# microsoft/DirectXTex

Measured on AMD Instinct MI355X. Metric: Mtexels/s BC7 encode (4096^2 RGBA8, TEX_COMPRESS_DEFAULT), higher is better.
Workload: dtype fp32 seed fit + i32 exact error sums (u8 texels in, 128-bit blocks out); 1 GPU; cfg2: 4096x4096 RGBA8 -> BC7_UNORM, TEX_COMPRESS_DEFAULT, one image per GPU, source and payload resident in HBM (dxtex_compress_device)

## Files before the change

directxtex_amd/csrc/bc6h_encode.hip:

```cpp
#include "dxtex_kernels.h"
#include "bc67_tables.h"
#include "bc7_core.h"
#include "bc6h_core.h"
#include "search_common.h"
#include <algorithm>
#include <cstdlib>
#include <cstdio>
#include <vector>

namespace dxtex
{
namespace
{
using namespace bc6h;

struct Ep16 { uint32_t a01, a2b0, b12; };
__device__ __forceinline__ Ep16 pack_ep16(const int (&A)[3], const int (&B)[3])
{
    Ep16 e;
    e.a01 = (uint32_t(A[0]) & 0xFFFFu) | (uint32_t(A[1]) << 16);
    e.a2b0 = (uint32_t(A[2]) & 0xFFFFu) | (uint32_t(B[0]) << 16);
    e.b12 = (uint32_t(B[1]) & 0xFFFFu) | (uint32_t(B[2]) << 16);
    return e;
}
// ... 14 lines not shown
__device__ __forceinline__ PkState pk_pack(const Perturb6& s)
{
    PkState p; p.ep = pack_ep16(s.ep.A, s.ep.B); p.err = s.err; p.err0 = s.err0;
    p.misc = (uint32_t(s.new0) & 0xFFFFu) | (uint32_t(s.ch) << 16) | (uint32_t(s.sub) << 18) | (uint32_t(s.do_b) << 20);
    return p;
}
__device__ __forceinline__ Perturb6 pk_unpack(const PkState& p, bool sg)
{
    Perturb6 s; unpack_ep16(p.ep, sg, s.ep.A, s.ep.B); s.err = p.err; s.err0 = p.err0;
    s.new0 = int(int16_t(p.misc & 0xFFFFu)); s.ch = int((p.misc >> 16) & 3u); s.sub = int((p.misc >> 18) & 3u); s.do_b = int((p.misc >> 20) & 1u);
    return s;
}
struct Rec6 { Ep16 ep; float err; };
struct Best6 { float err; uint32_t mode; uint64_t lo, hi; };
struct OrgSave { Ep16 ep; float err; uint64_t idx; };
struct OptSave { uint64_t idx; float err; uint32_t swapped; };

enum : int { SEED_INTS = 17 * 6 + 2 };

struct Bc6hArgs
{
    SegTable seg;
    uint32_t nblocks;
    int isSigned;
    int prune;
    uint32_t taskBase;
    int prec1[4];
    float* fpix;
    uint8_t* lists;
    int* seeds;
    Rec6* recs;
    OrgSave* orgs;
    uint2* order; uint32_t* tinfo; uint32_t* counters;
    Best6* best;
    float* bounds;
    int boundsReady;
    int filterStats;
    int samePrec;
    struct OptSave* opts;
    int saveOpt;
    ModeRt mode;
};

constexpr uint32_t kDoneBit6 = 1u << 23;

#if !defined(DXTEX_BC6H_DEFAULT_ORDER)
#define DXTEX_BC6H_DEFAULT_ORDER "5,6,7,8,0,2,3,4,1,9"
#endif

__device__ __forceinline__ Texels slot_texels(float* slot , int np)
{
    Texels t; t.r = slot; t.g = slot + 16 * 64; t.b = slot + 32 * 64; t.stride = 64; t.np = np;
    return t;
}

__device__ __forceinline__ int gather_texels(const float* planes, uint32_t mask, float* slot, uint64_t& pos)
{
    int np = 0; pos = 0;
#pragma unroll
    for (int i = 0; i < 16; ++i)
        if ((mask >> i) & 1u)
        {
            slot[np * 64] = planes[i]; slot[(16 + np) * 64] = planes[16 + i]; slot[(32 + np) * 64] = planes[32 + i];
            pos |= uint64_t(i) << (4 * np);
            ++np;
        }
// ... 901 lines not shown
        const float tr = gp[0], tg = gp[16], tb = gp[32];
        EndPts e;
        unpack_ep16(rec.ep, sg, e.A, e.B);
        Perturb6 st = perturb6_begin(e, rec.err);
        while (st.ch < 3)
        {
            float err; int v;
            perturb6_wave_macro(tr, tg, tb, lane, st, prec, sg, err, v);
            st = perturb6_transition(st, err, v);
        }
        if (lane == 0)
        {
            a.recs[myTask].ep = pack_ep16(st.ep.A, st.ep.B);
            { const float mk = ep16_mark(sg, st.ep.A, st.ep.B); if (mk < 0.0f) a.recs[myTask].err = mk; }
        }
    }
}

__global__ void __launch_bounds__(256) bc6h_store_kernel(Bc6hArgs a)
{
    const uint32_t nb = blockIdx.x * 256u + threadIdx.x;
    if (nb >= a.nblocks) return;
    const Best6 b = a.best[nb];
    const BcSeg& im = seg_of(a.seg, nb);
    const uint32_t gb = im.nb0 + (nb - im.l0);
    const uint32_t by = gb / im.nbw, bx = gb - by * im.nbw;
    uint64_t* out = reinterpret_cast<uint64_t*>(im.dst + uint64_t(by) * im.dstRowPitch) + 2 * uint64_t(bx);
    out[0] = b.lo; out[1] = b.hi;
}

const uint64_t kMaxBlocksPerPass6 = dev_env("DXTEX_MAX_BLOCKS_PER_PASS") ? std::max<uint64_t>(1, strtoull(dev_env("DXTEX_MAX_BLOCKS_PER_PASS"), nullptr, 10)) : (1u << 22);
struct Scratch6
{
    size_t fpix, lists, seeds, recs, orgs, order, tinfo, counters, best, bounds, recs1, orgs1, order1, tinfo1, counters1, opts, total;
    explicit Scratch6(uint64_t nb)
    {
        auto up = [](size_t v) { return (v + 255) & ~size_t(255); };
        size_t o = 0;
        fpix = o; o = up(o + nb * 48 * sizeof(float));
        lists = o; o = up(o + nb * 8);
        seeds = o; o = up(o + nb * SEED_INTS * sizeof(int));
        recs = o; o = up(o + nb * 16 * sizeof(Rec6));
        orgs = o; o = up(o + nb * 16 * sizeof(OrgSave));
        order = o; o = up(o + nb * 16 * sizeof(uint2));
        tinfo = o; o = up(o + nb * 16 * sizeof(uint32_t));
        counters = o; o = up(o + 128 * sizeof(uint32_t));
        best = o; o = up(o + nb * sizeof(Best6));
        bounds = o; o = up(o + nb * 17 * sizeof(float));
        recs1 = o; o = up(o + nb * 4 * sizeof(Rec6));
        orgs1 = o; o = up(o + nb * 4 * sizeof(OrgSave));
        order1 = o; o = up(o + nb * 4 * sizeof(uint2));
        tinfo1 = o; o = up(o + nb * 4 * sizeof(uint32_t));
        counters1 = o; o = up(o + 128 * sizeof(uint32_t));
        opts = o; o = up(o + nb * 16 * sizeof(OptSave));
        total = o;
    }
};
}

size_t bc6h_scratch_bytes(uint64_t nblocks, size_t nimages)
{
    return Scratch6(nblocks < kMaxBlocksPerPass6 ? nblocks : kMaxBlocksPerPass6).total + seg_table_bytes(nblocks, kMaxBlocksPerPass6, nimages);
}

hipError_t launch_bc6h_encode(const SrcView& src, uint8_t* dst, uint64_t dstRowPitch, bool isSigned, void* scratch,
                              hipStream_t stream, KernelMarks* marks, const SideStreams* side)
{
    BcImage one; one.src = src; one.dst = dst; one.dstRowPitch = dstRowPitch;
    return launch_bc6h_encode_many(&one, 1, isSigned, scratch, stream, marks, side);
}

hipError_t launch_bc6h_encode_many(const BcImage* images, size_t count, bool isSigned, void* scratch, hipStream_t stream, KernelMarks* marks,
                                   const SideStreams* side)
{
#define DXTEX_MARK(NAME) do { if (marks) marks->mark(NAME); } while (0)
    std::vector<BcSeg> segs;
    std::vector<BcPass> passes;
    uint64_t perPass = 0;
    if (!build_passes(images, count, kMaxBlocksPerPass6, segs, passes, &perPass)) return hipSuccess;
    const Scratch6 L(perPass);
    uint8_t* base = static_cast<uint8_t*>(scratch);
    BcSeg* dSegs = reinterpret_cast<BcSeg*>(base + L.total);
    const hipError_t ce = upload_segments(dSegs, segs, passes, stream);
    if (ce != hipSuccess) return ce;
    for (const BcPass& pass : passes)
    {
        Bc6hArgs a;
        set_pass(a.seg, dSegs, segs, pass);
        a.nblocks = pass.nblocks;
        a.isSigned = isSigned ? 1 : 0;
        static const bool noPrune = dev_env("DXTEX_BC6H_NO_PRUNE") != nullptr;
        a.prune = noPrune ? 0 : 1;
        a.fpix = reinterpret_cast<float*>(base + L.fpix);
        a.lists = base + L.lists;
        a.seeds = reinterpret_cast<int*>(base + L.seeds);
        a.recs = reinterpret_cast<Rec6*>(base + L.recs);
        a.orgs = reinterpret_cast<OrgSave*>(base + L.orgs);
        a.order = reinterpret_cast<uint2*>(base + L.order);
        a.tinfo = reinterpret_cast<uint32_t*>(base + L.tinfo);
        a.counters = reinterpret_cast<uint32_t*>(base + L.counters);
        a.best = reinterpret_cast<Best6*>(base + L.best);
        a.bounds = reinterpret_cast<float*>(base + L.bounds);
        a.opts = reinterpret_cast<OptSave*>(base + L.opts);
        a.saveOpt = 0;
        a.boundsReady = 0;
        a.filterStats = 0;
        a.mode = ModeRt();

        DXTEX_MARK("bc6h_rough");
        hipLaunchKernelGGL(bc6h_rough_kernel, dim3((a.nblocks + 3) / 4), dim3(256), 0, stream, a);
        DXTEX_MARK("bc6h_block_seed");
        hipLaunchKernelGGL(bc6h_block_seed_kernel, dim3((a.nblocks + 255) / 256), dim3(256), 0, stream, a);
        if (dev_env("DXTEX_BC6H_DUMP"))
        {
            (void)hipStreamSynchronize(stream);
            const uint32_t n = std::min<uint32_t>(a.nblocks, 4);
            std::vector<uint8_t> l(n * 8); std::vector<int> sd(n * SEED_INTS);
            (void)hipMemcpy(l.data(), a.lists, l.size(), hipMemcpyDeviceToHost);
            (void)hipMemcpy(sd.data(), a.seeds, sd.size() * 4, hipMemcpyDeviceToHost);
            for (uint32_t b = 0; b < n; ++b)
            {
                fprintf(stderr, "block %u shapes:", b);
                for (int i = 0; i < 8; ++i) fprintf(stderr, " %d", l[b * 8 + i]);
                fprintf(stderr, "\n  seeds rank0:");
                for (int i = 0; i < 12; ++i) fprintf(stderr, " %d", sd[b * SEED_INTS + i]);
                fprintf(stderr, "\n");
            }
        }
        static const int onlyMode = dev_env("DXTEX_BC6H_ONLY_MODE") ? atoi(dev_env("DXTEX_BC6H_ONLY_MODE")) : -1;
        static const bool noSearch = dev_env("DXTEX_BC6H_NO_SEARCH") != nullptr;
        static const Bc6hMode kModes[14] = {
            { 0x00, 1, 1, 3, { 10, 10, 10 }, { 5, 5, 5 } }, { 0x01, 1, 1, 3, { 7, 7, 7 }, { 6, 6, 6 } }, { 0x02, 1, 1, 3, { 11, 11, 11 }, { 5, 4, 4 } },
            { 0x06, 1, 1, 3, { 11, 11, 11 }, { 4, 5, 4 } }, { 0x0a, 1, 1, 3, { 11, 11, 11 }, { 4, 4, 5 } }, { 0x0e, 1, 1, 3, { 9, 9, 9 }, { 5, 5, 5 } },
            { 0x12, 1, 1, 3, { 8, 8, 8 }, { 6, 5, 5 } }, { 0x16, 1, 1, 3, { 8, 8, 8 }, { 5, 6, 5 } }, { 0x1a, 1, 1, 3, { 8, 8, 8 }, { 5, 5, 6 } },
            { 0x1e, 1, 0, 3, { 6, 6, 6 }, { 6, 6, 6 } }, { 0x03, 0, 0, 4, { 10, 10, 10 }, { 10, 10, 10 } }, { 0x07, 0, 1, 4, { 11, 11, 11 }, { 9, 9, 9 } },
            { 0x0b, 0, 1, 4, { 12, 12, 12 }, { 8, 8, 8 } }, { 0x0f, 0, 1, 4, { 16, 16, 16 }, { 4, 4, 4 } } };
        auto set_mode_on = [&](Bc6hArgs& a, int mi)
        {
            const Bc6hMode& k = kModes[mi];
            a.mode.index = mi; a.mode.code = k.code; a.mode.regions2 = k.regions2; a.mode.transformed = k.transformed; a.mode.prec = k.prec[0];
            for (int c = 0; c < 3; ++c) a.mode.delta[c] = k.delta[c];
        };
        auto set_mode = [&](int mi) { set_mode_on(a, mi); };
        auto sort_tasks = [&](const Bc6hArgs& a, uint32_t ntasks, hipStream_t stream)
        {
            const uint32_t binGroups = std::min<uint32_t>(kBinGroups, (ntasks + 255) / 256);
            (void)hipMemsetAsync(a.counters, 0, 128 * sizeof(uint32_t), stream);
            hipLaunchKernelGGL(bc7_bin_count_kernel, dim3(binGroups), dim3(256), 0, stream, a.tinfo, ntasks, a.counters);
            hipLaunchKernelGGL(bc7_bin_scan_kernel, dim3(1), dim3(1), 0, stream, a.counters);
            hipLaunchKernelGGL(bc7_bin_scatter_kernel, dim3(binGroups), dim3(256), 0, stream, a.tinfo, ntasks, a.counters, a.order);
        };
        a.taskBase = 0;
        for (int m = 0; m < 4; ++m) a.prec1[m] = kModes[10 + m].prec[0];
        static const std::vector<int> order6 = []
        {
            std::vector<int> o;
            const char* e = dev_env("DXTEX_BC6H_ORDER");
            const char* p = e ? e : DXTEX_BC6H_DEFAULT_ORDER;
            while (*p) { if (*p >= '0' && *p <= '9') o.push_back(int(strtol(p, const_cast<char**>(&p), 10))); else ++p; }
            return o;
        }();
        int prevPrec = -1;
        a.samePrec = 0;
        std::vector<int> run2;
        for (int mi : order6) if (mi >= 0 && mi <= 9 && (onlyMode < 0 || mi == onlyMode)) run2.push_back(mi);
        static const int forkBack = dev_env("DXTEX_BC6H_FORK_BACK") ? atoi(dev_env("DXTEX_BC6H_FORK_BACK")) : 2;
        const SideStreams* fork = (marks || forkBack <= 0 || run2.size() < size_t(forkBack) + 1 || onlyMode >= 0) ? nullptr : side;
        Bc6hArgs a1 = a;
        a1.recs = reinterpret_cast<Rec6*>(base + L.recs1);
        a1.orgs = reinterpret_cast<OrgSave*>(base + L.orgs1);
        a1.order = reinterpret_cast<uint2*>(base + L.order1);
        a1.tinfo = reinterpret_cast<uint32_t*>(base + L.tinfo1);
        a1.counters = reinterpret_cast<uint32_t*>(base + L.counters1);
        a1.samePrec = 0;
        auto one_region_search = [&](hipStream_t stream, KernelMarks* marks)
        {
            const uint32_t gridPP = (a1.nblocks + 255) / 256;
            DXTEX_MARK("bc6h_pre_1region");
            a1.boundsReady = 0;
            for (int m = 0; m < 4; ++m)
            {
                if (onlyMode >= 0 && 10 + m != onlyMode) continue;
                set_mode_on(a1, 10 + m); a1.taskBase = uint32_t(m) * a1.nblocks;
                hipLaunchKernelGGL(bc6h_pre_kernel<0>, dim3(gridPP), dim3(256), 0, stream, a1);
                a1.boundsReady = 1;
            }
            const uint32_t ntasks = a1.nblocks * 4u;
            if (onlyMode >= 0)
                for (int m = 0; m < 4; ++m) if (10 + m != onlyMode) (void)hipMemsetAsync(a1.tinfo + uint64_t(m) * a1.nblocks, 0, uint64_t(a1.nblocks) * 4, stream);
            DXTEX_MARK("bc6h_bin_1region");
            sort_tasks(a1, ntasks, stream);
            DXTEX_MARK("bc6h_perturb_1region");
            static const uint32_t waveMax = dev_env("DXTEX_BC6H_WAVE_MAX") ? uint32_t(strtoul(dev_env("DXTEX_BC6H_WAVE_MAX"), nullptr, 0)) : kWaveTaskMax6;
            if (!noSearch)
            {
                hipLaunchKernelGGL(bc6h_perturb_kernel<16>, dim3(std::min<uint32_t>(kSearchWaves, (ntasks + 63) / 64)), dim3(64), 0, stream, a1, waveMax);
                hipLaunchKernelGGL(bc6h_perturb_wave_kernel, dim3(std::min<uint32_t>(kSearchWaves, ntasks)), dim3(64), 0, stream, a1, waveMax);
            }
        };
        bool forked = false;
        for (size_t at = 0; at < run2.size(); ++at)
        {
            const int mi = run2[at];
            if (fork && at + size_t(forkBack) == run2.size())
            {
                (void)hipEventRecord(fork->forked, stream);
// ... 84 lines not shown
```

directxtex_amd/csrc/bc7_encode.hip:

```cpp
#include "dxtex_kernels.h"
#include "bc67_tables.h"
#include "bc7_core.h"
#include "search_common.h"
#include <algorithm>
#include <cstdio>
#include <cstdlib>
#include <vector>

namespace dxtex
{
namespace
{
using namespace bc7;

struct Cand { uint32_t err; uint32_t ord; uint64_t lo, hi; };

enum : int { SLOT_M0 = 0, SLOT_M1, SLOT_M2, SLOT_M3, SLOT_M4A, SLOT_M4B, SLOT_M5, SLOT_M6, SLOT_M7, NUM_SLOTS };
enum : int { LIST_BYTES = 64 };

enum : int { PHASE_ALL = 0, PHASE_EARLY = 1, PHASE_LATE = 2 };

struct Bc7Args
{
    SegTable seg;
    uint32_t nblocks;
    uint32_t flags;
    uint8_t* lists;
    Cand* cands;
    uint32_t* px;
    struct TaskRec* recs;
    uint2* order;
    uint32_t* tinfo;
    uint32_t* counters;
    uint32_t* zeroOrd;
    uint2* seeds1;
    uint2* seeds3;
    uint2* seeds;
    int* bestErr;
    int prune;
    const uint32_t* flagged;
    uint32_t early6Min;
    uint32_t earlyAlphaMin;
    int early6Pct;
    int phase;
    const uint32_t* gate;
    uint32_t gateMin;
    uint32_t perturbWaveMax;
    uint32_t exhWaveMax;
};

constexpr uint32_t kWaveTaskMax = 262144;
constexpr uint32_t kWaveTaskMax45 = 24576;
constexpr uint32_t kPerturbWaveMax = 32768;

__device__ __forceinline__ void load_block_texel(const SrcView& src, uint32_t nbw, uint32_t nb, uint32_t t, float* f4, uint32_t& ldr)
{
    const uint32_t by = nb / nbw, bx = nb - by * nbw;
    const uint32_t x0 = bx * 4, y0 = by * 4;
    const uint32_t pw = min(4u, src.width - x0), ph = min(4u, src.height - y0);
    const uint32_t sx = x0 + replicate_src(t & 3, pw), sy = y0 + replicate_src(t >> 2, ph);
    const Texel px = convert_texel(load_texel(src.pixels + uint64_t(sy) * src.rowPitch, sx, src.format), src.tcv, src.tsw);
    f4[0] = px.r; f4[1] = px.g; f4[2] = px.b; f4[3] = px.a;
    const float c[4] = { px.r, px.g, px.b, px.a };
    ldr = 0;
#pragma unroll
    for (int i = 0; i < 4; ++i)
// ... 1207 lines not shown

__global__ void __launch_bounds__(256) bc7_pick_kernel(Bc7Args a, uint32_t slotMask)
{
    const uint32_t nb = blockIdx.x * 256u + threadIdx.x;
    if (nb >= a.nblocks) return;
    const Cand* c = a.cands + uint64_t(nb) * NUM_SLOTS;
    uint64_t bestKey = ~0ull;
    uint64_t lo = 0, hi = 0;
#pragma unroll
    for (int s = 0; s < NUM_SLOTS; ++s)
    {
        if (!((slotMask >> s) & 1u)) continue;
        if (s == SLOT_M7 && a.flagged[1] == 0) continue;
        const Cand v = c[s];
        if (v.err == 0xFFFFFFFFu) continue;
        const uint64_t key = (uint64_t(v.err) << 32) | v.ord;
        if (key < bestKey) { bestKey = key; lo = v.lo; hi = v.hi; }
    }
    const BcSeg& sg = seg_of(a.seg, nb);
    const uint32_t gb = sg.nb0 + (nb - sg.l0);
    const uint32_t by = gb / sg.nbw, bx = gb - by * sg.nbw;
    uint64_t* out = reinterpret_cast<uint64_t*>(sg.dst + uint64_t(by) * sg.dstRowPitch) + 2 * uint64_t(bx);
    out[0] = lo; out[1] = hi;
}
}

namespace
{
const uint64_t kMaxBlocksPerPass = dev_env("DXTEX_MAX_BLOCKS_PER_PASS") ? std::max<uint64_t>(1, strtoull(dev_env("DXTEX_MAX_BLOCKS_PER_PASS"), nullptr, 10)) : (1u << 22);
constexpr int kMaxTasksPerBlock = 64;
const uint64_t kSmallPassBlocks = dev_env("DXTEX_BC7_SMALL_BLOCKS") ? strtoull(dev_env("DXTEX_BC7_SMALL_BLOCKS"), nullptr, 10) : 262144;
struct ScratchLayout
{
    size_t lists, cands, px, recs, order, tinfo, counters, zeroOrd, bestErr, seeds, seeds1, seeds3, flagcnt, auxRecs, auxOrder, auxTinfo, auxCounters, total;
    size_t auxTpb, auxSlices;
    explicit ScratchLayout(uint64_t nb, bool threeSubsets)
    {
        auto up = [](size_t v) { return (v + 255) & ~size_t(255); };
        const size_t tpb = threeSubsets ? kMaxTasksPerBlock : 32;
        const bool small = nb <= kSmallPassBlocks;
        auxTpb = small ? tpb : 4; auxSlices = small ? size_t(kSideStreams) : 2;
        size_t o = 0;
        lists = o; o = up(o + nb * LIST_BYTES);
        cands = o; o = up(o + nb * NUM_SLOTS * sizeof(Cand));
        px = o; o = up(o + nb * 64);
        recs = o; o = up(o + nb * tpb * sizeof(TaskRec));
        order = o; o = up(o + nb * tpb * sizeof(uint2));
        tinfo = o; o = up(o + nb * tpb * sizeof(uint32_t));
        counters = o; o = up(o + 64 * sizeof(uint32_t));
        zeroOrd = o; o = up(o + nb * sizeof(uint32_t));
        bestErr = o; o = up(o + nb * sizeof(int));
        seeds = o; o = up(o + nb * 64 * sizeof(uint2));
        seeds1 = o; o = up(o + nb * 2 * sizeof(uint2));
        seeds3 = o; o = up(o + (threeSubsets ? nb * 192 * sizeof(uint2) : 0));
        flagcnt = o; o = up(o + 256);
        auxRecs = o; o = up(o + auxSlices * nb * auxTpb * sizeof(TaskRec));
        auxOrder = o; o = up(o + auxSlices * nb * auxTpb * sizeof(uint2));
        auxTinfo = o; o = up(o + auxSlices * nb * auxTpb * sizeof(uint32_t));
        auxCounters = o; o = up(o + size_t(kSideStreams) * 64 * sizeof(uint32_t));
        total = o;
    }
};

template<int MODE, int IM>
void launch_mode(const Bc7Args& a0, hipStream_t stream, KernelMarks* marks, const char* const (&names)[7])
{
    typedef TaskMap<MODE, IM> TM;
    constexpr int BPW = (TM::TPB >= 64) ? 1 : 64 / TM::TPB;
    const uint32_t nb = a0.nblocks;
    const uint32_t ntasks = nb * uint32_t(TM::TPB);
    const uint32_t gridPP = (nb + 4 * BPW - 1) / (4 * BPW);
    constexpr bool kWhole = TM::NS == 1;
    constexpr uint32_t kExhMax = (MODE == 6) ? kWaveTaskMax : kWaveTaskMax45;
    static const bool noGroup = dev_env("DXTEX_BC7_NO_GROUP") != nullptr;
    const bool maybeShortP = kWhole && !noGroup && (MODE == 6 || ntasks <= 4u * kPerturbWaveMax);
    const bool maybeShortE = kWhole && !noGroup && (MODE == 6 || ntasks <= 4u * kExhMax);
    const uint32_t wavesP = std::min<uint32_t>(kSearchWaves, (ntasks + 1) / 2), wavesE = std::min<uint32_t>(kSearchWaves, ntasks);
    Bc7Args a = a0;
    a.gate = nullptr; a.gateMin = 0;
    if (a0.flagged && !(a0.flags & BCF_BC7_QUICK))
    {
        if (MODE == 7) { a.gate = a0.flagged + 1; a.gateMin = 1; }
        else if (a0.phase == PHASE_EARLY && (MODE == 4 || MODE == 5)) { a.gate = a0.flagged + 1; a.gateMin = std::max<uint32_t>(1u, a0.earlyAlphaMin); }
        else if (a0.phase == PHASE_EARLY && MODE == 6) { a.gate = a0.flagged; a.gateMin = std::max<uint32_t>(1u, a0.early6Min); }
    }
    a.perturbWaveMax = maybeShortP ? kPerturbWaveMax : 0u;
    a.exhWaveMax = maybeShortE ? kExhMax : 0u;
    if (marks) marks->mark(names[0]);
    hipLaunchKernelGGL((bc7_pre_kernel<MODE, IM>), dim3(gridPP), dim3(256), 0, stream, a);
    if (marks) marks->mark(names[1]);
    (void)hipMemsetAsync(a.counters, 0, 64 * sizeof(uint32_t), stream);
    const uint32_t binGroups = std::min<uint32_t>(kBinGroups, (ntasks + 255) / 256);
    hipLaunchKernelGGL(bc7_bin_count_kernel, dim3(binGroups), dim3(256), 0, stream, a.tinfo, ntasks, a.counters, a.gate, a.gateMin);
    hipLaunchKernelGGL(bc7_bin_scan_kernel, dim3(1), dim3(1), 0, stream, a.counters);
    hipLaunchKernelGGL(bc7_bin_scatter_kernel, dim3(binGroups), dim3(256), 0, stream, a.tinfo, ntasks, a.counters, a.order, a.gate, a.gateMin);
    if (marks) marks->mark(names[2]);
    const uint32_t waves = std::min<uint32_t>(kSearchWaves, (ntasks + 63) / 64);
    static const int tailBelow = dev_env("DXTEX_BC7_TAIL_BELOW") ? atoi(dev_env("DXTEX_BC7_TAIL_BELOW")) : 48;
    static const bool perturbPlain = dev_env("DXTEX_BC7_PERTURB_PLAIN") != nullptr;
    static const int rangeTests = dev_env("DXTEX_BC7_NO_PEEL") ? 3 : ((dev_env("DXTEX_BC7_RANGE_TESTS") ? atoi(dev_env("DXTEX_BC7_RANGE_TESTS")) & 0xFF : DXTEX_RANGE_TESTS) |
                                                                       ((dev_env("DXTEX_BC7_PEEL_LAYERS") ? atoi(dev_env("DXTEX_BC7_PEEL_LAYERS")) : 1) << 8));
    if constexpr (PaletteBits<MODE, IM>::AB == 0)
    {
        if constexpr (MODE == 1 || MODE == 6)
        {
            if (perturbPlain) hipLaunchKernelGGL((bc7_perturb_kernel<MODE, IM, CH_ALL>), dim3(waves), dim3(64), 0, stream, a, 0);
            else hipLaunchKernelGGL((bc7_perturb_filter_kernel<MODE, IM, CH_ALL>), dim3(waves), dim3(64), 0, stream, a, 0);
        }
        else
            hipLaunchKernelGGL((bc7_perturb_kernel<MODE, IM, CH_ALL>), dim3(waves), dim3(64), 0, stream, a, 0);
        if constexpr (kWhole) { if (maybeShortP) hipLaunchKernelGGL((bc7_perturb_wave_kernel<MODE, IM, CH_ALL>), dim3(wavesP), dim3(64), 0, stream, a); }
        if (marks) marks->mark(names[4]);
        if constexpr (kWhole) { if (maybeShortE) hipLaunchKernelGGL((bc7_exhaustive_wave_kernel<MODE, IM, CH_ALL>), dim3(wavesE), dim3(64), 0, stream, a); }
        hipLaunchKernelGGL((bc7_exhaustive_kernel<MODE, IM, CH_ALL>), dim3(waves), dim3(64), 0, stream, a, 1, tailBelow, rangeTests);
    }
    else
    {
        if constexpr (MODE == 4 && IM == 1 && DXTEX_PF_M4 != 0)
        {
            if (perturbPlain) hipLaunchKernelGGL((bc7_perturb_kernel<MODE, IM, CH_COLOR>), dim3(waves), dim3(64), 0, stream, a, 0);
            else hipLaunchKernelGGL((bc7_perturb_filter_kernel<MODE, IM, CH_COLOR>), dim3(waves), dim3(64), 0, stream, a, 0);
        }
        else
            hipLaunchKernelGGL((bc7_perturb_kernel<MODE, IM, CH_COLOR>), dim3(waves), dim3(64), 0, stream, a, 0);
        if (maybeShortP) hipLaunchKernelGGL((bc7_perturb_wave_kernel<MODE, IM, CH_COLOR>), dim3(wavesP), dim3(64), 0, stream, a);
        if (marks) marks->mark(names[3]);
        hipLaunchKernelGGL((bc7_perturb_kernel<MODE, IM, CH_ALPHA>), dim3(waves), dim3(64), 0, stream, a, 1);
        if (maybeShortP) hipLaunchKernelGGL((bc7_perturb_wave_kernel<MODE, IM, CH_ALPHA>), dim3(wavesP), dim3(64), 0, stream, a);
// ... 104 lines not shown
                                  const SideStreams* side)
{
#define DXTEX_MARK(NAME) do { if (marks) marks->mark(NAME); } while (0)
#define DXTEX_MODE(MODE, IM, TAG) do { static const char* const n_[7] = { "bc7_pre_" TAG, "bc7_bin_" TAG, "bc7_perturb_" TAG, "bc7_perturb_alpha_" TAG, \
                                           "bc7_exhaustive_" TAG, "bc7_exhaustive_alpha_" TAG, "bc7_post_" TAG }; \
                                       launch_mode<MODE, IM>(a, stream, marks, n_); } while (0)
    std::vector<BcSeg> segs;
    std::vector<BcPass> passes;
    uint64_t perPass = 0;
    if (!build_passes(images, count, kMaxBlocksPerPass, segs, passes, &perPass)) return hipSuccess;
    const bool three = (flags & BCF_USE_3SUBSETS) != 0;
    const ScratchLayout L(perPass, three);
    uint8_t* base = static_cast<uint8_t*>(scratch);
    BcSeg* dSegs = reinterpret_cast<BcSeg*>(base + L.total);
    const hipError_t ce = upload_segments(dSegs, segs, passes, stream);
    if (ce != hipSuccess) return ce;
    const bool quick = (flags & BCF_BC7_QUICK) != 0;

    for (const BcPass& pass : passes)
    {
        Bc7Args a;
        set_pass(a.seg, dSegs, segs, pass);
        a.nblocks = pass.nblocks;
        a.flags = flags;
        a.perturbWaveMax = 0; a.exhWaveMax = 0;
        a.gate = nullptr; a.gateMin = 0;
        a.lists = base + L.lists;
        a.cands = reinterpret_cast<Cand*>(base + L.cands);
        a.px = reinterpret_cast<uint32_t*>(base + L.px);
        a.recs = reinterpret_cast<TaskRec*>(base + L.recs);
        a.order = reinterpret_cast<uint2*>(base + L.order);
        a.tinfo = reinterpret_cast<uint32_t*>(base + L.tinfo);
        a.counters = reinterpret_cast<uint32_t*>(base + L.counters);
        a.zeroOrd = reinterpret_cast<uint32_t*>(base + L.zeroOrd);
        a.bestErr = reinterpret_cast<int*>(base + L.bestErr);
        a.seeds = reinterpret_cast<uint2*>(base + L.seeds);
        a.seeds1 = reinterpret_cast<uint2*>(base + L.seeds1);
        a.seeds3 = reinterpret_cast<uint2*>(base + L.seeds3);
        static const bool noPrune = dev_env("DXTEX_BC7_NO_PRUNE") != nullptr;
        a.prune = noPrune ? 0 : 1;
        static const int early6 = dev_env("DXTEX_BC7_EARLY6_PCT") ? atoi(dev_env("DXTEX_BC7_EARLY6_PCT")) : 100;
        a.early6Pct = early6;
        uint32_t slotMask = 0;

        uint32_t* flagCount = reinterpret_cast<uint32_t*>(base + L.flagcnt);
        a.flagged = flagCount;
        static const int early6MinPct = dev_env("DXTEX_BC7_EARLY6_MIN_PCT") ? atoi(dev_env("DXTEX_BC7_EARLY6_MIN_PCT")) : -1;
        static const int earlyAlphaMinPct = dev_env("DXTEX_BC7_EARLYA_MIN_PCT") ? atoi(dev_env("DXTEX_BC7_EARLYA_MIN_PCT")) : 25;
        const bool smallPlanRuns = side && !marks && !quick && dev_env("DXTEX_BC7_SERIAL") == nullptr && dev_env("DXTEX_BC7_NO_SMALL_PLAN") == nullptr &&
                                   L.auxTpb >= 32 && perPass <= kSmallPassBlocks && dev_env("DXTEX_BC7_ORDER") == nullptr;
        a.early6Min = uint32_t(uint64_t(a.nblocks) * uint32_t(early6MinPct >= 0 ? early6MinPct : (smallPlanRuns ? 25 : 50)) / 100u);
        a.earlyAlphaMin = uint32_t(uint64_t(a.nblocks) * uint32_t(earlyAlphaMinPct) / 100u);
        if (!quick)
        {
            DXTEX_MARK("bc7_rough");
            hipLaunchKernelGGL(bc7_rough_kernel, dim3((a.nblocks + 3) / 4), dim3(256), 0, stream, a);
            (void)hipMemsetAsync(flagCount, 0, 256, stream);
            hipLaunchKernelGGL(bc7_flag_count_kernel, dim3((a.nblocks + 255) / 256), dim3(256), 0, stream, a, flagCount);
        }
        else
        {
            DXTEX_MARK("bc7_texels");
            hipLaunchKernelGGL(bc7_texels_kernel, dim3((a.nblocks * 16 + 255) / 256), dim3(256), 0, stream, a);
        }
        DXTEX_MARK("bc7_block_seeds");
        if (!quick) hipLaunchKernelGGL(bc7_block_seeds_kernel<false>, dim3((a.nblocks + 255) / 256), dim3(256), 0, stream, a);
// ... 17 lines not shown
            a.phase = (step >= 20) ? PHASE_LATE : (step >= 10) ? PHASE_EARLY : PHASE_ALL;
            switch (step)
            {
            case 0: DXTEX_MODE(0, 0, "mode0"); slotMask |= 1u << SLOT_M0; break;
            case 1: DXTEX_MODE(1, 0, "mode1"); slotMask |= 1u << SLOT_M1; break;
            case 2: DXTEX_MODE(2, 0, "mode2"); slotMask |= 1u << SLOT_M2; break;
            case 3: DXTEX_MODE(3, 0, "mode3"); slotMask |= 1u << SLOT_M3; break;
            case 4: DXTEX_MODE(4, 0, "mode4_im0"); slotMask |= 1u << SLOT_M4A; break;
            case 14: DXTEX_MODE(4, 0, "mode4_im0_early"); slotMask |= 1u << SLOT_M4A; break;
            case 24: DXTEX_MODE(4, 0, "mode4_im0_late"); slotMask |= 1u << SLOT_M4A; break;
            case 8: DXTEX_MODE(4, 1, "mode4_im1"); slotMask |= 1u << SLOT_M4B; break;
            case 18: DXTEX_MODE(4, 1, "mode4_im1_early"); slotMask |= 1u << SLOT_M4B; break;
            case 28: DXTEX_MODE(4, 1, "mode4_im1_late"); slotMask |= 1u << SLOT_M4B; break;
            case 5: DXTEX_MODE(5, 0, "mode5"); slotMask |= 1u << SLOT_M5; break;
            case 15: DXTEX_MODE(5, 0, "mode5_early"); slotMask |= 1u << SLOT_M5; break;
            case 25: DXTEX_MODE(5, 0, "mode5_late"); slotMask |= 1u << SLOT_M5; break;
            case 6: DXTEX_MODE(6, 0, "mode6"); slotMask |= 1u << SLOT_M6; break;
            case 16: DXTEX_MODE(6, 0, "mode6_early"); slotMask |= 1u << SLOT_M6; break;
            case 26: DXTEX_MODE(6, 0, "mode6_late"); slotMask |= 1u << SLOT_M6; break;
            case 7: DXTEX_MODE(7, 0, "mode7"); slotMask |= 1u << SLOT_M7; break;
            default: break;
            }
        };
        auto family45 = [](int step) { const int m = step % 10; return m == 4 || m == 8 || m == 5; };
        static const bool serial45 = dev_env("DXTEX_BC7_SERIAL") != nullptr;
        const SideStreams* fork = (marks || serial45 || quick) ? nullptr : side;
        auto side_args = [&](const Bc7Args& a0, size_t k)
        {
            Bc7Args b = a0;
            b.recs = reinterpret_cast<TaskRec*>(base + L.auxRecs) + k * size_t(a0.nblocks) * L.auxTpb;
            b.order = reinterpret_cast<uint2*>(base + L.auxOrder) + k * size_t(a0.nblocks) * L.auxTpb;
            b.tinfo = reinterpret_cast<uint32_t*>(base + L.auxTinfo) + k * size_t(a0.nblocks) * L.auxTpb;
            b.counters = reinterpret_cast<uint32_t*>(base + L.auxCounters) + k * 64;
            return b;
        };
        static const std::vector<std::vector<std::vector<int>>> smallPlan = []
        {
            const char* e = dev_env("DXTEX_BC7_SMALL_PLAN");
            const char* p = e ? e : "1,26/3,2/16,14,15,18,7,0|24/28/25";
            std::vector<std::vector<std::vector<int>>> stages(1, std::vector<std::vector<int>>(1));
            while (*p)
            {
                if (*p >= '0' && *p <= '9') stages.back().back().push_back(int(strtol(p, const_cast<char**>(&p), 10)));
                else
                {
                    if (*p == '|') stages.emplace_back(1);
                    else if (*p == '/' && stages.back().size() < size_t(kSideStreams) + 1) stages.back().emplace_back();
                    ++p;
                }
            }
            return stages;
        }();
        static const bool noSmall = dev_env("DXTEX_BC7_NO_SMALL_PLAN") != nullptr;
        if (fork && !noSmall && smallPlanRuns)
        {
            for (const std::vector<std::vector<int>>& stage : smallPlan)
            {
                if (stage.size() > 1) (void)hipEventRecord(fork->forked, stream);
                for (size_t l = 1; l < stage.size(); ++l)
                {
                    hipStream_t s = fork->side[l - 1];
                    (void)hipStreamWaitEvent(s, fork->forked, 0);
                    const Bc7Args al = side_args(a, l - 1);
                    for (int step : stage[l])
                        if (three || (step != 0 && step != 2)) run_step(step, al, s, nullptr);
                    (void)hipEventRecord(fork->joined[l - 1], s);
// ... 9 lines not shown
            const int step = order[at];
            if (!three && (step == 0 || step == 2)) { ++at; continue; }
            size_t run = 1;
            if (fork && family45(step))
                while (at + run < order.size() && run < 3 && family45(order[at + run]) && order[at + run] / 10 == step / 10) ++run;
            if (run == 1) { run_step(step, a, stream, marks); ++at; continue; }
            (void)hipEventRecord(fork->forked, stream);
            for (size_t k = 1; k < run; ++k)
            {
                const Bc7Args b = side_args(a, k - 1);
                (void)hipStreamWaitEvent(fork->side[k - 1], fork->forked, 0);
                run_step(order[at + k], b, fork->side[k - 1], nullptr);
                (void)hipEventRecord(fork->joined[k - 1], fork->side[k - 1]);
            }
            run_step(step, a, stream, nullptr);
            for (size_t k = 1; k < run; ++k) (void)hipStreamWaitEvent(stream, fork->joined[k - 1], 0);
            at += run;
        }
#if defined(DXTEX_EXH_STATS)
        hipLaunchKernelGGL(bc7_stats_print_kernel, dim3(1), dim3(1), 0, stream, reinterpret_cast<unsigned long long*>(flagCount) + 4);
#endif
        DXTEX_MARK("bc7_pick");
        hipLaunchKernelGGL(bc7_pick_kernel, dim3((a.nblocks + 255) / 256), dim3(256), 0, stream, a, slotMask);
    }
    DXTEX_MARK(nullptr);
#undef DXTEX_MODE
#undef DXTEX_MARK
#if defined(DXTEX_BC7_WAVETIMES)
    bc7_wavetimes_report();
#endif
    return hipGetLastError();
}
}
```

directxtex_amd/csrc/search_common.h:

```cpp
#pragma once
#include <hip/hip_runtime.h>
#include <stdint.h>
#include <algorithm>
#include <cstring>
#include <vector>
#include "dxtex_kernels.h"

namespace dxtex
{
namespace
{
struct BcSeg
{
    SrcView src;
    uint8_t* dst;
    uint64_t dstRowPitch;
    uint32_t nbw;
    uint32_t nb0;
    uint32_t l0;
    uint32_t pad;
};

struct SegTable
{
// ... 90 lines not shown
}

__device__ __forceinline__ int wave_prefix_min(int v)
{
    v = min(v, __builtin_amdgcn_update_dpp(v, v, 0x111, 0xF, 0xF, false));
    v = min(v, __builtin_amdgcn_update_dpp(v, v, 0x112, 0xF, 0xF, false));
    v = min(v, __builtin_amdgcn_update_dpp(v, v, 0x114, 0xF, 0xF, false));
    v = min(v, __builtin_amdgcn_update_dpp(v, v, 0x118, 0xF, 0xF, false));
    v = min(v, __builtin_amdgcn_update_dpp(v, v, 0x142, 0xA, 0xF, false));
    v = min(v, __builtin_amdgcn_update_dpp(v, v, 0x143, 0xC, 0xF, false));
    return v;
}

__device__ __forceinline__ void selection_pass(int& e, uint32_t& s, int lane, int i)
{
    const int v = (lane >= i) ? e : 0x7FFFFFFF;
    const int incl = wave_prefix_min(v);
    int excl = __builtin_amdgcn_update_dpp(0x7FFFFFFF, incl, 0x138, 0xF, 0xF, false);
    if (lane <= i) excl = 0x7FFFFFFF;
    const bool isrec = (lane > i) && (e < excl);
    const unsigned long long mask = __ballot(isrec);
    int srcLane = lane;
    if (isrec)
    {
        const unsigned long long below = mask & ((1ull << lane) - 1ull);
        srcLane = below ? (63 - __clzll(below)) : i;
    }
    else if (lane == i && mask)
        srcLane = 63 - __clzll(mask);
    e = __shfl(e, srcLane);
    s = uint32_t(__shfl(int(s), srcLane));
}

constexpr int kBinGroups = 2048;

__global__ void __launch_bounds__(256) bc7_bin_count_kernel(const uint32_t* tinfo, uint32_t ntasks, uint32_t* counters, const uint32_t* gate = nullptr, uint32_t gateMin = 0)
{
    if (gate && *gate < gateMin) return;
    __shared__ uint32_t hist[17];
    if (threadIdx.x < 17) hist[threadIdx.x] = 0;
    __syncthreads();
    const uint32_t per = (ntasks + gridDim.x - 1) / gridDim.x;
    const uint32_t t0 = blockIdx.x * per, t1 = min(ntasks, t0 + per);
    for (uint32_t t = t0 + threadIdx.x; t < t1; t += 256)
    {
        const uint32_t np = tinfo[t] >> 24;
        if (np) atomicAdd(&hist[np], 1u);
    }
    __syncthreads();
    if (threadIdx.x >= 1 && threadIdx.x <= 16 && hist[threadIdx.x]) atomicAdd(&counters[threadIdx.x], hist[threadIdx.x]);
}

__global__ void bc7_bin_scan_kernel(uint32_t* counters)
{
    if (threadIdx.x != 0 || blockIdx.x != 0) return;
    uint32_t run = 0;
    for (int b = 16; b >= 1; --b) { counters[17 + b] = run; run += counters[b]; }
    counters[34] = run;
}

__global__ void __launch_bounds__(256) bc7_bin_scatter_kernel(const uint32_t* tinfo, uint32_t ntasks, uint32_t* counters, uint2* order, const uint32_t* gate = nullptr, uint32_t gateMin = 0)
{
    if (gate && *gate < gateMin) return;
    __shared__ uint32_t hist[17], cursor[17];
    if (threadIdx.x < 17) hist[threadIdx.x] = 0;
    __syncthreads();
    const uint32_t per = (ntasks + gridDim.x - 1) / gridDim.x;
    const uint32_t t0 = blockIdx.x * per, t1 = min(ntasks, t0 + per);
    for (uint32_t t = t0 + threadIdx.x; t < t1; t += 256)
    {
        const uint32_t np = tinfo[t] >> 24;
        if (np) atomicAdd(&hist[np], 1u);
    }
    __syncthreads();
    if (threadIdx.x >= 1 && threadIdx.x <= 16)
        cursor[threadIdx.x] = hist[threadIdx.x] ? atomicAdd(&counters[17 + threadIdx.x], hist[threadIdx.x]) : 0u;
    __syncthreads();
    for (uint32_t t = t0 + threadIdx.x; t < t1; t += 256)
    {
        const uint32_t ti = tinfo[t], np = ti >> 24;
        if (np) order[atomicAdd(&cursor[np], 1u)] = make_uint2(t, ti);
    }
}

constexpr int kQueueBase = 36;
constexpr int kSearchWaves = 8192;

constexpr uint32_t kQueueBatch = 128;

struct WaveQueue
{
    uint32_t lo, hi;
    bool drained;
};

__device__ __forceinline__ uint32_t queue_take(WaveQueue& q, uint32_t* head, uint32_t live, unsigned long long idle, int lane)
{
    if (q.lo >= q.hi && !q.drained)
    {
        const uint32_t batch = (live > uint32_t(kSearchWaves) * 64u) ? kQueueBatch : 64u;
        uint32_t base = 0;
        if (lane == 0) base = atomicAdd(head, batch);
        base = uint32_t(__builtin_amdgcn_readfirstlane(int(base)));
        q.lo = base;
        q.hi = min(base + batch, live);
        if (base >= live) { q.drained = true; q.hi = q.lo; }
    }
    const uint32_t k = uint32_t(__popcll(idle & ((1ull << lane) - 1ull)));
    const uint32_t avail = q.hi - q.lo;
    const uint32_t mine = (((idle >> lane) & 1ull) && k < avail) ? (q.lo + k) : 0xFFFFFFFFu;
    q.lo += min(uint32_t(__popcll(idle)), avail);
    return mine;
}

}
// ... 2 lines not shown
```

Baseline: 136.4 Mtexels/s.

## Replace atomic task binning with deterministic per-wave histogram counting sort

Replaces the shared/global atomic-based count/scan/scatter bin sort of search tasks with a wave-level counting sort. Each wave counts bins by ballot, writes a per-wave histogram, a single 1024-thread kernel scans it, and the scatter uses mbcnt ranks for stable, atomic-free placement. This also drops the memset launch. The aim is to cut atomic contention and launch overhead in the sort step between search phases. The cost is extra scratch for the per-wave histograms and a serial single-block scan.

```diff
diff --git a/directxtex_amd/csrc/bc6h_encode.hip b/directxtex_amd/csrc/bc6h_encode.hip
--- a/directxtex_amd/csrc/bc6h_encode.hip
+++ b/directxtex_amd/csrc/bc6h_encode.hip
@@ -70,6 +70,7 @@
     Rec6* recs;
     OrgSave* orgs;
     uint2* order; uint32_t* tinfo; uint32_t* counters;
+    uint32_t* binHist;
     Best6* best;
     float* bounds;
     int boundsReady;
@@ -1037,7 +1038,7 @@
 const uint64_t kMaxBlocksPerPass6 = dev_env("DXTEX_MAX_BLOCKS_PER_PASS") ? std::max<uint64_t>(1, strtoull(dev_env("DXTEX_MAX_BLOCKS_PER_PASS"), nullptr, 10)) : (1u << 22);
 struct Scratch6
 {
-    size_t fpix, lists, seeds, recs, orgs, order, tinfo, counters, best, bounds, recs1, orgs1, order1, tinfo1, counters1, opts, total;
+    size_t fpix, lists, seeds, recs, orgs, order, tinfo, counters, best, bounds, recs1, orgs1, order1, tinfo1, counters1, opts, binHist, binHist1, total;
     explicit Scratch6(uint64_t nb)
     {
         auto up = [](size_t v) { return (v + 255) & ~size_t(255); };
@@ -1058,6 +1059,8 @@
         tinfo1 = o; o = up(o + nb * 4 * sizeof(uint32_t));
         counters1 = o; o = up(o + 128 * sizeof(uint32_t));
         opts = o; o = up(o + nb * 16 * sizeof(OptSave));
+        binHist = o; o = up(o + sort_hist_words(nb * 16) * sizeof(uint32_t));
+        binHist1 = o; o = up(o + sort_hist_words(nb * 4) * sizeof(uint32_t));
         total = o;
     }
 };
@@ -1104,6 +1107,7 @@
         a.order = reinterpret_cast<uint2*>(base + L.order);
         a.tinfo = reinterpret_cast<uint32_t*>(base + L.tinfo);
         a.counters = reinterpret_cast<uint32_t*>(base + L.counters);
+        a.binHist = reinterpret_cast<uint32_t*>(base + L.binHist);
         a.best = reinterpret_cast<Best6*>(base + L.best);
         a.bounds = reinterpret_cast<float*>(base + L.bounds);
         a.opts = reinterpret_cast<OptSave*>(base + L.opts);
@@ -1149,11 +1153,10 @@
         auto set_mode = [&](int mi) { set_mode_on(a, mi); };
         auto sort_tasks = [&](const Bc6hArgs& a, uint32_t ntasks, hipStream_t stream)
         {
-            const uint32_t binGroups = std::min<uint32_t>(kBinGroups, (ntasks + 255) / 256);
-            (void)hipMemsetAsync(a.counters, 0, 128 * sizeof(uint32_t), stream);
-            hipLaunchKernelGGL(bc7_bin_count_kernel, dim3(binGroups), dim3(256), 0, stream, a.tinfo, ntasks, a.counters);
-            hipLaunchKernelGGL(bc7_bin_scan_kernel, dim3(1), dim3(1), 0, stream, a.counters);
-            hipLaunchKernelGGL(bc7_bin_scatter_kernel, dim3(binGroups), dim3(256), 0, stream, a.tinfo, ntasks, a.counters, a.order);
+#if defined(DXTEX_DEV)
+            if (dev_env("DXTEX_BC6H_STATS")) (void)hipMemsetAsync(a.counters + 64, 0, 64 * sizeof(uint32_t), stream);
+#endif
+            launch_task_sort(a.tinfo, ntasks, a.counters, a.binHist, a.order, nullptr, 0, stream);
         };
         a.taskBase = 0;
         for (int m = 0; m < 4; ++m) a.prec1[m] = kModes[10 + m].prec[0];
@@ -1177,6 +1180,7 @@
         a1.order = reinterpret_cast<uint2*>(base + L.order1);
         a1.tinfo = reinterpret_cast<uint32_t*>(base + L.tinfo1);
         a1.counters = reinterpret_cast<uint32_t*>(base + L.counters1);
+        a1.binHist = reinterpret_cast<uint32_t*>(base + L.binHist1);
         a1.samePrec = 0;
         auto one_region_search = [&](hipStream_t stream, KernelMarks* marks)
         {
diff --git a/directxtex_amd/csrc/bc7_encode.hip b/directxtex_amd/csrc/bc7_encode.hip
--- a/directxtex_amd/csrc/bc7_encode.hip
+++ b/directxtex_amd/csrc/bc7_encode.hip
@@ -32,6 +32,7 @@
     uint2* order;
     uint32_t* tinfo;
     uint32_t* counters;
+    uint32_t* binHist;
     uint32_t* zeroOrd;
     uint2* seeds1;
     uint2* seeds3;
@@ -1305,7 +1306,7 @@
 const uint64_t kSmallPassBlocks = dev_env("DXTEX_BC7_SMALL_BLOCKS") ? strtoull(dev_env("DXTEX_BC7_SMALL_BLOCKS"), nullptr, 10) : 262144;
 struct ScratchLayout
 {
-    size_t lists, cands, px, recs, order, tinfo, counters, zeroOrd, bestErr, seeds, seeds1, seeds3, flagcnt, auxRecs, auxOrder, auxTinfo, auxCounters, total;
+    size_t lists, cands, px, recs, order, tinfo, counters, zeroOrd, bestErr, seeds, seeds1, seeds3, flagcnt, auxRecs, auxOrder, auxTinfo, auxCounters, binHist, auxBinHist, histWords, auxHistWords, total;
     size_t auxTpb, auxSlices;
     explicit ScratchLayout(uint64_t nb, bool threeSubsets)
     {
@@ -1331,6 +1332,9 @@
         auxOrder = o; o = up(o + auxSlices * nb * auxTpb * sizeof(uint2));
         auxTinfo = o; o = up(o + auxSlices * nb * auxTpb * sizeof(uint32_t));
         auxCounters = o; o = up(o + size_t(kSideStreams) * 64 * sizeof(uint32_t));
+        histWords = sort_hist_words(nb * tpb); auxHistWords = sort_hist_words(nb * auxTpb);
+        binHist = o; o = up(o + histWords * sizeof(uint32_t));
+        auxBinHist = o; o = up(o + size_t(kSideStreams) * auxHistWords * sizeof(uint32_t));
         total = o;
     }
 };
@@ -1362,11 +1366,7 @@
     if (marks) marks->mark(names[0]);
     hipLaunchKernelGGL((bc7_pre_kernel<MODE, IM>), dim3(gridPP), dim3(256), 0, stream, a);
     if (marks) marks->mark(names[1]);
-    (void)hipMemsetAsync(a.counters, 0, 64 * sizeof(uint32_t), stream);
-    const uint32_t binGroups = std::min<uint32_t>(kBinGroups, (ntasks + 255) / 256);
-    hipLaunchKernelGGL(bc7_bin_count_kernel, dim3(binGroups), dim3(256), 0, stream, a.tinfo, ntasks, a.counters, a.gate, a.gateMin);
-    hipLaunchKernelGGL(bc7_bin_scan_kernel, dim3(1), dim3(1), 0, stream, a.counters);
-    hipLaunchKernelGGL(bc7_bin_scatter_kernel, dim3(binGroups), dim3(256), 0, stream, a.tinfo, ntasks, a.counters, a.order, a.gate, a.gateMin);
+    launch_task_sort(a.tinfo, ntasks, a.counters, a.binHist, a.order, a.gate, a.gateMin, stream);
     if (marks) marks->mark(names[2]);
     const uint32_t waves = std::min<uint32_t>(kSearchWaves, (ntasks + 63) / 64);
     static const int tailBelow = dev_env("DXTEX_BC7_TAIL_BELOW") ? atoi(dev_env("DXTEX_BC7_TAIL_BELOW")) : 48;
@@ -1537,6 +1537,7 @@
         a.order = reinterpret_cast<uint2*>(base + L.order);
         a.tinfo = reinterpret_cast<uint32_t*>(base + L.tinfo);
         a.counters = reinterpret_cast<uint32_t*>(base + L.counters);
+        a.binHist = reinterpret_cast<uint32_t*>(base + L.binHist);
         a.zeroOrd = reinterpret_cast<uint32_t*>(base + L.zeroOrd);
         a.bestErr = reinterpret_cast<int*>(base + L.bestErr);
         a.seeds = reinterpret_cast<uint2*>(base + L.seeds);
@@ -1620,6 +1621,7 @@
             b.order = reinterpret_cast<uint2*>(base + L.auxOrder) + k * size_t(a0.nblocks) * L.auxTpb;
             b.tinfo = reinterpret_cast<uint32_t*>(base + L.auxTinfo) + k * size_t(a0.nblocks) * L.auxTpb;
             b.counters = reinterpret_cast<uint32_t*>(base + L.auxCounters) + k * 64;
+            b.binHist = reinterpret_cast<uint32_t*>(base + L.auxBinHist) + k * L.auxHistWords;
             return b;
         };
         static const std::vector<std::vector<std::vector<int>>> smallPlan = []
@@ -1695,3 +1697,29 @@
     return hipGetLastError();
 }
 }
+
+#if defined(DXTEX_DEV)
+extern "C" __attribute__((visibility("default"))) int dxtex_dev_task_sort(const uint32_t* tinfo, uint32_t ntasks, const uint32_t* gate, uint32_t gateMin,
+                                                                         uint64_t* orderOut, uint32_t* countersOut)
+{
+    using namespace dxtex;
+    const size_t histBytes = sort_hist_words(ntasks) * sizeof(uint32_t), orderBytes = std::max<size_t>(ntasks, 1) * sizeof(uint2), ctrBytes = 64 * sizeof(uint32_t);
+    uint8_t* scratch = nullptr;
+    hipError_t e = hipMalloc(reinterpret_cast<void**>(&scratch), histBytes + orderBytes + ctrBytes);
+    if (e != hipSuccess) return int(e);
+    uint32_t* hist = reinterpret_cast<uint32_t*>(scratch);
+    uint2* order = reinterpret_cast<uint2*>(scratch + histBytes);
+    uint32_t* counters = reinterpret_cast<uint32_t*>(scratch + histBytes + orderBytes);
+    e = hipMemsetAsync(scratch, 0xFF, histBytes + orderBytes + ctrBytes, nullptr);
+    if (e == hipSuccess)
+    {
+        launch_task_sort(tinfo, ntasks, counters, hist, order, gate, gateMin, nullptr);
+        e = hipGetLastError();
+    }
+    if (e == hipSuccess) e = hipStreamSynchronize(nullptr);
+    if (e == hipSuccess && ntasks) e = hipMemcpy(orderOut, order, size_t(ntasks) * sizeof(uint2), hipMemcpyDeviceToHost);
+    if (e == hipSuccess) e = hipMemcpy(countersOut, counters, ctrBytes, hipMemcpyDeviceToHost);
+    (void)hipFree(scratch);
+    return int(e);
+}
+#endif
diff --git a/directxtex_amd/csrc/search_common.h b/directxtex_amd/csrc/search_common.h
--- a/directxtex_amd/csrc/search_common.h
+++ b/directxtex_amd/csrc/search_common.h
@@ -146,55 +146,162 @@
     s = uint32_t(__shfl(int(s), srcLane));
 }
 
-constexpr int kBinGroups = 2048;
-
-__global__ void __launch_bounds__(256) bc7_bin_count_kernel(const uint32_t* tinfo, uint32_t ntasks, uint32_t* counters, const uint32_t* gate = nullptr, uint32_t gateMin = 0)
+__device__ __forceinline__ uint32_t wave_prefix_sum(uint32_t x)
+{
+    int v = int(x);
+    v += __builtin_amdgcn_update_dpp(0, v, 0x111, 0xF, 0xF, false);
+    v += __builtin_amdgcn_update_dpp(0, v, 0x112, 0xF, 0xF, false);
+    v += __builtin_amdgcn_update_dpp(0, v, 0x114, 0xF, 0xF, false);
+    v += __builtin_amdgcn_update_dpp(0, v, 0x118, 0xF, 0xF, false);
+    v += __builtin_amdgcn_update_dpp(0, v, 0x142, 0xA, 0xF, false);
+    v += __builtin_amdgcn_update_dpp(0, v, 0x143, 0xC, 0xF, false);
+    return uint32_t(v);
+}
+
+constexpr int kSortWaves = 8192;
+
+inline uint32_t sort_waves(uint64_t ntasks) { return uint32_t(std::max<uint64_t>(1, std::min<uint64_t>(kSortWaves, (ntasks + 63) / 64))); }
+__host__ __device__ inline uint32_t sort_row_stride(uint32_t W) { return (W + 3u) & ~3u; }
+inline size_t sort_hist_words(uint64_t ntasks) { return size_t(16) * sort_row_stride(sort_waves(ntasks)); }
+
+__device__ __forceinline__ void sort_slice(uint32_t ntasks, uint32_t w, uint32_t W, uint32_t& s0, uint32_t& s1)
+{
+    const uint32_t steps = (ntasks + 63u) >> 6, per = (steps + W - 1u) / W;
+    s0 = min(steps, w * per); s1 = min(steps, s0 + per);
+}
+
+constexpr int kSortBatch = 4;
+
+__global__ void __launch_bounds__(64) task_sort_count_kernel(const uint32_t* __restrict__ tinfo, uint32_t ntasks, uint32_t* __restrict__ binHist,
+                                                             const uint32_t* gate = nullptr, uint32_t gateMin = 0)
 {
     if (gate && *gate < gateMin) return;
-    __shared__ uint32_t hist[17];
-    if (threadIdx.x < 17) hist[threadIdx.x] = 0;
+    const uint32_t lane = threadIdx.x, w = blockIdx.x, W = gridDim.x;
+    uint32_t s0, s1;
+    sort_slice(ntasks, w, W, s0, s1);
+    uint32_t count = 0;
+    for (uint32_t s = s0; s < s1; s += kSortBatch)
+    {
+        uint32_t np[kSortBatch];
+#pragma unroll
+        for (int k = 0; k < kSortBatch; ++k)
+        {
+            const uint32_t t = (s + k) * 64u + lane;
+            np[k] = (s + k < s1 && t < ntasks) ? tinfo[t] >> 24 : 0u;
+        }
+#pragma unroll
+        for (int k = 0; k < kSortBatch; ++k)
+        {
+            unsigned long long todo = __ballot(np[k] != 0u);
+            while (todo)
+            {
+                const uint32_t b = uint32_t(__builtin_amdgcn_readlane(int(np[k]), __builtin_ctzll(todo)));
+                const unsigned long long m = __ballot(np[k] == b);
+                if (lane == b) count += uint32_t(__popcll(m));
+                todo &= ~m;
+            }
+        }
+    }
+    if (lane >= 1 && lane <= 16) binHist[(16u - lane) * sort_row_stride(W) + w] = count;
+}
+
+__global__ void __launch_bounds__(1024) task_sort_scan_kernel(uint32_t* __restrict__ binHist, uint32_t W, uint32_t* __restrict__ counters,
+                                                              const uint32_t* gate = nullptr, uint32_t gateMin = 0)
+{
+    const uint32_t tid = threadIdx.x, lane = tid & 63u, row = tid >> 6;
+    if (tid >= 35 && tid < 64) counters[tid] = 0;
+    if (gate && *gate < gateMin)
+    {
+        if (tid < 35) counters[tid] = 0;
+        return;
+    }
+    __shared__ uint32_t rowTotal[16];
+    const uint32_t stride = sort_row_stride(W), quads = stride >> 2;
+    uint4* rowp = reinterpret_cast<uint4*>(binHist + row * stride);
+    auto load = [&](uint32_t q)
+    {
+        uint4 x = make_uint4(0, 0, 0, 0);
+        if (q < quads)
+        {
+            x = rowp[q];
+            const uint32_t e = q * 4u;
+            if (e + 1u >= W) x.y = 0;
+            if (e + 2u >= W) x.z = 0;
+            if (e + 3u >= W) x.w = 0;
+        }
+        return x;
+    };
+    uint32_t sum = 0;
+    for (uint32_t q = lane; q < quads; q += 64u) { const uint4 x = load(q); sum += x.x + x.y + x.z + x.w; }
+    const uint32_t total = uint32_t(__builtin_amdgcn_readlane(int(wave_prefix_sum(sum)), 63));
+    if (lane == 0) rowTotal[row] = total;
     __syncthreads();
-    const uint32_t per = (ntasks + gridDim.x - 1) / gridDim.x;
-    const uint32_t t0 = blockIdx.x * per, t1 = min(ntasks, t0 + per);
-    for (uint32_t t = t0 + threadIdx.x; t < t1; t += 256)
-    {
-        const uint32_t np = tinfo[t] >> 24;
-        if (np) atomicAdd(&hist[np], 1u);
-    }
-    __syncthreads();
-    if (threadIdx.x >= 1 && threadIdx.x <= 16 && hist[threadIdx.x]) atomicAdd(&counters[threadIdx.x], hist[threadIdx.x]);
-}
-
-__global__ void bc7_bin_scan_kernel(uint32_t* counters)
-{
-    if (threadIdx.x != 0 || blockIdx.x != 0) return;
-    uint32_t run = 0;
-    for (int b = 16; b >= 1; --b) { counters[17 + b] = run; run += counters[b]; }
-    counters[34] = run;
-}
-
-__global__ void __launch_bounds__(256) bc7_bin_scatter_kernel(const uint32_t* tinfo, uint32_t ntasks, uint32_t* counters, uint2* order, const uint32_t* gate = nullptr, uint32_t gateMin = 0)
+    uint32_t carry = 0;
+    for (uint32_t r = 0; r < row; ++r) carry += rowTotal[r];
+    if (lane == 0)
+    {
+        const uint32_t b = 16u - row;
+        counters[b] = total; counters[17u + b] = carry;
+        if (row == 15) { counters[34] = carry + total; counters[0] = 0; counters[17] = 0; }
+    }
+    for (uint32_t q0 = 0; q0 < quads; q0 += 64u)
+    {
+        const uint32_t q = q0 + lane;
+        const uint4 x = load(q);
+        const uint32_t mine = x.x + x.y + x.z + x.w;
+        const uint32_t incl = wave_prefix_sum(mine);
+        const uint32_t excl = carry + incl - mine;
+        if (q < quads) rowp[q] = make_uint4(excl, excl + x.x, excl + x.x + x.y, excl + x.x + x.y + x.z);
+        carry += uint32_t(__builtin_amdgcn_readlane(int(incl), 63));
+    }
+}
+
+__global__ void __launch_bounds__(64) task_sort_scatter_kernel(const uint32_t* __restrict__ tinfo, uint32_t ntasks, const uint32_t* __restrict__ binBase,
+                                                               uint2* __restrict__ order, const uint32_t* gate = nullptr, uint32_t gateMin = 0)
 {
     if (gate && *gate < gateMin) return;
-    __shared__ uint32_t hist[17], cursor[17];
-    if (threadIdx.x < 17) hist[threadIdx.x] = 0;
-    __syncthreads();
-    const uint32_t per = (ntasks + gridDim.x - 1) / gridDim.x;
-    const uint32_t t0 = blockIdx.x * per, t1 = min(ntasks, t0 + per);
-    for (uint32_t t = t0 + threadIdx.x; t < t1; t += 256)
-    {
-        const uint32_t np = tinfo[t] >> 24;
-        if (np) atomicAdd(&hist[np], 1u);
-    }
-    __syncthreads();
-    if (threadIdx.x >= 1 && threadIdx.x <= 16)
-        cursor[threadIdx.x] = hist[threadIdx.x] ? atomicAdd(&counters[17 + threadIdx.x], hist[threadIdx.x]) : 0u;
-    __syncthreads();
-    for (uint32_t t = t0 + threadIdx.x; t < t1; t += 256)
-    {
-        const uint32_t ti = tinfo[t], np = ti >> 24;
-        if (np) order[atomicAdd(&cursor[np], 1u)] = make_uint2(t, ti);
-    }
+    const uint32_t lane = threadIdx.x, w = blockIdx.x, W = gridDim.x;
+    uint32_t s0, s1;
+    sort_slice(ntasks, w, W, s0, s1);
+    if (s0 >= s1) return;
+    uint32_t next = 0;
+    if (lane >= 1 && lane <= 16) next = binBase[(16u - lane) * sort_row_stride(W) + w];
+    for (uint32_t s = s0; s < s1; s += kSortBatch)
+    {
+        uint32_t ti[kSortBatch];
+#pragma unroll
+        for (int k = 0; k < kSortBatch; ++k)
+        {
+            const uint32_t t = (s + k) * 64u + lane;
+            ti[k] = (s + k < s1 && t < ntasks) ? tinfo[t] : 0u;
+        }
+#pragma unroll
+        for (int k = 0; k < kSortBatch; ++k)
+        {
+            const uint32_t np = ti[k] >> 24;
+            unsigned long long todo = __ballot(np != 0u);
+            uint32_t pos = 0;
+            while (todo)
+            {
+                const uint32_t b = uint32_t(__builtin_amdgcn_readlane(int(np), __builtin_ctzll(todo)));
+                const unsigned long long m = __ballot(np == b);
+                const uint32_t first = uint32_t(__builtin_amdgcn_readlane(int(next), int(b)));
+                if (np == b) pos = first + __builtin_amdgcn_mbcnt_hi(uint32_t(m >> 32), __builtin_amdgcn_mbcnt_lo(uint32_t(m), 0u));
+                if (lane == b) next += uint32_t(__popcll(m));
+                todo &= ~m;
+            }
+            if (np) order[pos] = make_uint2((s + k) * 64u + lane, ti[k]);
+        }
+    }
+}
+
+inline void launch_task_sort(const uint32_t* tinfo, uint32_t ntasks, uint32_t* counters, uint32_t* binHist, uint2* order,
+                             const uint32_t* gate, uint32_t gateMin, hipStream_t stream)
+{
+    const uint32_t W = sort_waves(ntasks);
+    hipLaunchKernelGGL(task_sort_count_kernel, dim3(W), dim3(64), 0, stream, tinfo, ntasks, binHist, gate, gateMin);
+    hipLaunchKernelGGL(task_sort_scan_kernel, dim3(1), dim3(1024), 0, stream, binHist, W, counters, gate, gateMin);
+    hipLaunchKernelGGL(task_sort_scatter_kernel, dim3(W), dim3(64), 0, stream, tinfo, ntasks, static_cast<const uint32_t*>(binHist), order, gate, gateMin);
 }
 
 constexpr int kQueueBase = 36;
```

New measurement: 136.7 Mtexels/s (median of 6 runs). About the same (+0.2%).
